# balkce/beamform

Measured on AMD Instinct MI355X. Metric: stft_frames_per_sec, higher is better.
Workload: dtype f64; 1 GPU; das 8-mic 1024-pt (hop 512), 65536-frame batch per GPU, 1 stream(s), planar input resident in HBM; frames_per_gpu=65536, frames_fed_per_gpu=65536, mics=8, fft=1024, hop=512, streams=1, layout=planar, gather=n/a, parallelism=independent batches x1, input=uniform noise in [-0.5, 0.5), settle_launches_before_warmup=408, forward_transforms_per_frame_pair=6

## Files before the change

beamform_amd/csrc/das_f64_w64.hip:

```cpp
#include <hip/hip_runtime.h>

#include <type_traits>

#include "launch_trace.hpp"
#include "pipeline_kernels.hpp"
#include "w64_f64_dev.hpp"

namespace bf {

namespace {

constexpr int kBlock = 512;
constexpr int kWaves = kBlock / 64;
constexpr int kHop = 512;
constexpr int kTwD = 2 * (1024 + 4 * kTw2RowW64Rot);
constexpr int oTw = 0;
constexpr int oPlane = kTwD;
constexpr int oGain = oPlane + kWaves * kPlaneD;
constexpr int oCross = oGain + 4 * 2048;
constexpr int oFlag = oCross + 512;
constexpr int kWinRow = 18;
constexpr int oWin = oFlag + 8;
constexpr int kLdsD = oWin + 64 * kWinRow;

// ... 218 lines not shown
            }
        } else {
            const float *parea = (pw < kWaves - 1) ? reinterpret_cast<const float *>(lds + oPlane + pw * kPlaneD) : s_cross + ((it + 1) & 1) * kHop;
            while (s_ready[pw] < (int)(t - 1)) __builtin_amdgcn_s_sleep(1);
            asm volatile("" ::: "memory");
            float prev[8];
#pragma unroll
            for (int j = 0; j < 8; ++j) prev[j] = parea[64 * j + lane];
            asm volatile("" ::: "memory");
            if (lane == 0) s_cons[pw] = (int)(t - 1);
#pragma unroll
            for (int j = 0; j < 8; ++j) yo[(unsigned)(64 * j + lane)] = prev[j] + o[j];
        }
        if (t == T1 - 1) {
            if (T1 < a.n_frames) {
                float *yn = ys + T1 * kHop;
#pragma unroll
                for (int j = 0; j < 8; ++j) atomicAdd(yn + (unsigned)(64 * j + lane), o[j + 8]);
            } else {
                float *to = a.tail_out + (long)stream * kHop;
#pragma unroll
                for (int j = 0; j < 8; ++j) to[(unsigned)(64 * j + lane)] = o[j + 8];
            }
        }
    }
}


#ifdef BF_PARK_PLAIN
#define BF_PARK_LD(p) (*(const volatile float *)(p))
#else
#define BF_PARK_LD(p) __builtin_nontemporal_load(p)
#endif
constexpr int kGRow = 65;
constexpr int kGMic = 8 * kGRow;
constexpr int kSlots = 64;
constexpr int kTwP = 2 * (960 + 4 * kTw2RowW64Rot);
constexpr int pTw = 0;
constexpr int pPlane = kTwP;
constexpr int pGain = pPlane + kWaves * kPlaneD;
constexpr int pFlag = pGain + 7 * kGMic * 2;
constexpr int kRingR = 32;
constexpr int kRingSlots = kRingR + kWaves;
constexpr int pRing = pFlag + (kSlots + 4) / 2;
constexpr int pWin = pRing + kRingR / 2;
constexpr int kLdsP = pWin + 64 * kWinRow;
static_assert(kLdsP * 8 <= 160 * 1024, "LDS");
static_assert((pGain & 1) == 0 && (pWin & 1) == 0, "16-byte alignment");


typedef volatile __attribute__((address_space(3))) int *lds_int_t;
typedef volatile __attribute__((address_space(3))) unsigned long long *lds_u64_t;
__device__ __forceinline__ int lds_fetch_add(lds_int_t p, int v, int lane) {
    int old = 0;
    if (lane == 0) old = __hip_atomic_fetch_add((__attribute__((address_space(3))) int *)p, v, __ATOMIC_RELAXED, __HIP_MEMORY_SCOPE_WORKGROUP);
    return __builtin_amdgcn_readfirstlane(old);
}
__device__ __forceinline__ unsigned long long lds_fetch_add64(lds_u64_t p, int lane) {
    unsigned long long old = 0;
    if (lane == 0) old = __hip_atomic_fetch_add((__attribute__((address_space(3))) unsigned long long *)p, 1ull, __ATOMIC_RELAXED, __HIP_MEMORY_SCOPE_WORKGROUP);
    const unsigned lo = (unsigned)__builtin_amdgcn_readfirstlane((int)(unsigned)old), hi = (unsigned)__builtin_amdgcn_readfirstlane((int)(unsigned)(old >> 32));
    return ((unsigned long long)hi << 32) | lo;
}
struct DasSched {
    const int4 *chunks;
    unsigned *counter;
    int n_chunks;
};
__device__ __forceinline__ unsigned long long pack_work(unsigned vbase, int chunk, int pairs, int next) {
    return ((unsigned long long)(vbase & 0xFFFFFFu) << 40) | ((unsigned long long)(unsigned)chunk << 20) | ((unsigned long long)(unsigned)pairs << 10) | (unsigned)next;
}
struct PairWork {
    int4 d;
    int pos;
    int len;
    unsigned u;
    bool have;
};
__device__ __forceinline__ int4 load_chunk(const int4 *chunks, int k) {
    const int4 d = chunks[k];
// ... 96 lines not shown
    __builtin_amdgcn_wave_barrier();
}

__device__ __forceinline__ float max3abs(float m, float x, float y) {
#if defined(__HIP_DEVICE_COMPILE__)
    float r;
    asm("v_max3_f32 %0, %1, |%2|, |%3|" : "=v"(r) : "v"(m), "v"(x), "v"(y));
    return r;
#else
    return fmaxf(m, fmaxf(fabsf(x), fabsf(y)));
#endif
}

template <int LAYOUT>
__device__ __forceinline__ void das_f64_pair_body(const DasF64Args &a, const DasSched &sc) {
    __shared__ __attribute__((aligned(16))) double lds[kLdsP];
    const cx<double> *s_tw1 = reinterpret_cast<const cx<double> *>(lds + pTw) - 64;
    const cx<double> *s_tw2 = reinterpret_cast<const cx<double> *>(lds + pTw) + 960;
    const cx<double> *s_gain = reinterpret_cast<const cx<double> *>(lds + pGain);
    lds_int_t s_state = (lds_int_t)(lds + pFlag);
    lds_u64_t s_work = (lds_u64_t)(lds + pFlag + kSlots / 2);
    lds_int_t s_ring = (lds_int_t)(lds + pRing);
    (void)s_ring;

    const int tid = threadIdx.x, lane = tid & 63;
    const int w = __builtin_amdgcn_readfirstlane(tid >> 6);
    const int M = a.n_mics;
    double *plane = lds + pPlane + w * kPlaneD;
    double *wcol = plane + w64_col_rot(lane);
    double *row16 = plane + (lane & 15) * kRS + 16 * (lane >> 4);
    const double *wrow = lds + pWin + lane * kWinRow;
    typedef double cxa __attribute__((ext_vector_type(2)));
    typedef const __attribute__((address_space(3))) cxa *lds_gain_t;
    unsigned gd0 = (unsigned)(size_t)(lds_gain_t)(s_gain + lane);
    asm volatile("" : "+v"(gd0));
    gd0 &= ~15u;
    const unsigned g_mirror = 2u * (unsigned)(size_t)(lds_gain_t)s_gain + 1024u;

    float n0[8], n1[8], n2[8];
#ifndef BF_PAIR_NT
#define BF_PAIR_NT 0
#endif
    auto request = [&](const float *h0, const float *h1, const float *h2) {
#pragma unroll
        for (int j = 0; j < 8; ++j) {
            n0[j] = (BF_PAIR_NT & 2) ? __builtin_nontemporal_load(h0 + (unsigned)(64 * j + lane)) : h0[(unsigned)(64 * j + lane)];
            n1[j] = (BF_PAIR_NT & 1) ? __builtin_nontemporal_load(h1 + (unsigned)(64 * j + lane)) : h1[(unsigned)(64 * j + lane)];
            n2[j] = (BF_PAIR_NT & 4) ? __builtin_nontemporal_load(h2 + (unsigned)(64 * j + lane)) : h2[(unsigned)(64 * j + lane)];
        }
    };
    auto request_pair_mic = [&](int stream, long tA, int m) {
        const float *h1 = a.x + (long)stream * a.stream_stride_x + (long)m * a.mic_stride + tA * kHop;
        const float *h0 = tA >= 1 ? h1 - kHop : a.hist + ((long)stream * M + m) * kHop;
        const float *h2 = tA + 1 < a.n_frames ? h1 + kHop : h1;
        request(h0, h1, h2);
    };
    float q0[8], q1[8], q2[8];
    const double inv_m = 1.0 / (double)M;
    float e0[8], e1[8], e2[8];
    const int NT = a.n_tr, XM = a.extra_mic;
    auto request_extra = [&](bool on, int stream, long tA) {
        if (!on) {
#pragma unroll
            for (int j = 0; j < 8; ++j) e0[j] = e1[j] = e2[j] = 0.f;
            return;
        }
        const float *h1 = a.x + (long)stream * a.stream_stride_x + (long)XM * a.mic_stride + tA * kHop;
        const float *h0 = tA >= 1 ? h1 - kHop : a.hist + ((long)stream * M + XM) * kHop;
        const float *h2 = tA + 1 < a.n_frames ? h1 + kHop : h1;
#pragma unroll
// ... 90 lines not shown
#pragma unroll
        for (int j = 0; j < 8; ++j) {
            e0[j] = r.h[XM * kHop + (unsigned)(64 * j + lane)];
            e1[j] = r.a[XM * kHop + (unsigned)(64 * j + lane)];
            e2[j] = r.b[XM * kHop + (unsigned)(64 * j + lane)];
        }
    };
    RingHops curR{nullptr, nullptr, nullptr};
    (void)curR;

    BF_STAMP(0);
#ifdef BF_W64_STAMPS
    if (lane == 0 && blockIdx.x < 256) g_stamps[(blockIdx.x * 8 + w) * 64 + 59] = __builtin_amdgcn_s_memtime();
#endif
    PairWork cur;
    cur.d = load_chunk(sc.chunks, (int)blockIdx.x);
    cur.len = (cur.d.z + 1) >> 1;
    const int n_static = cur.len < kWaves ? cur.len : kWaves;
    cur.pos = w;
    cur.u = (unsigned)w;
    cur.have = w < n_static;
    if (LAYOUT == 0 && cur.have) {
        request_pair_mic(cur.d.x, cur.d.y + 2L * w, a.slot_mic[0]);
        request_extra(XM >= 0, cur.d.x, cur.d.y + 2L * w);
    } else {
        request_extra(false, 0, 0);
    }
    {
        const f64x2 *tw2 = a.tw + 64;
        f64x2 *ltw = reinterpret_cast<f64x2 *>(lds + pTw), *lg = reinterpret_cast<f64x2 *>(lds + pGain);
#pragma unroll 4
        for (int i = tid; i < kTwP / 2; i += kBlock) ltw[i] = tw2[i];
        for (int k = 0; k < NT; ++k) {
            const f64x2 *g2 = a.gains_mic + a.slot_mic[k] * kGMic;
#pragma unroll 2
            for (int i = tid; i < kGMic; i += kBlock) lg[k * kGMic + i] = g2[i];
        }
#pragma unroll 2
        for (int i = tid; i < 1024; i += kBlock) lds[pWin + (i & 63) * kWinRow + (i >> 6)] = a.win[i];
        if (tid < kSlots) s_state[tid] = 0;
        if (tid < kRingR) s_ring[tid] = 0;
        if (tid == 0) *s_work = pack_work(0u, (int)blockIdx.x, cur.len, n_static);
    }
    __syncthreads();
    BF_STAMP(1);
    BF_STATS_DECL;
    int it = 0;
    if (!cur.have) {
        cur = draw_pair(s_work, sc, lane, cur.d);
        if (LAYOUT == 0 && cur.have) {
            request_pair_mic(cur.d.x, cur.d.y + 2L * cur.pos, a.slot_mic[0]);
            request_extra(XM >= 0, cur.d.x, cur.d.y + 2L * cur.pos);
        }
    }
    int mode = 0;
    PairWork nxt;
    nxt.have = false;
    nxt.d = int4{0, 0, 0, 0};
    nxt.pos = nxt.len = 0;
    nxt.u = 0;
    while (cur.have) {
        if constexpr (LAYOUT == 1) {
            if (mode == 0) curR = prepare_pair(cur);
            request_ring_mic(curR, a.slot_mic[0]);
            request_ring_extra(XM >= 0, curR);
        }
        const int stream = cur.d.x;
        const long T0 = cur.d.y, T1 = T0 + cur.d.z;
        const long tA = T0 + 2L * cur.pos;
// ... 60 lines not shown
                if (mode == 2) {
#pragma unroll
                    for (int j = 0; j < 16; ++j) re[j] = 0.0;
                } else {
#pragma unroll
                    for (int j = 0; j < 16; ++j) im[j] = 0.0;
                }
            }
            if (k + 1 < NT) {
                if constexpr (LAYOUT == 1) request_ring_mic(curR, a.slot_mic[k + 1]);
                else request_pair_mic(stream, tA, a.slot_mic[k + 1]);
            } else {
                if (mode == 0) nxt = draw_pair(s_work, sc, lane, cur.d);
                if constexpr (LAYOUT == 0) {
                    if (mode != 1) {
                        if (nxt.have) request_pair_mic(nxt.d.x, nxt.d.y + 2L * nxt.pos, a.slot_mic[0]);
                        else request_pair_mic(stream, tA, a.slot_mic[0]);
                    }
                }
            }
            cx<double> tw[15];
            BF_STAGE();
            load_tw1<1, 9>(tw, s_tw1, lane);
            BF_STAGE();
            fft16_core<double, -1, true, 1>(re, im);
            BF_STAGE();
            load_tw1<9, 16>(tw, s_tw1, lane);
            BF_STAGE();
            mul_tw<false, 1, 9>(re, im, tw);
            BF_STAGE();
            mul_tw<false, 9, 16>(re, im, tw);
            BF_STAGE();
            T1_fwd(re, im, wcol, row16);
            load_tw2<1, 9>(tw, s_tw2, lane);
            BF_STAGE();
            fft16_core<double, -1, true>(re, im);
            BF_STAGE();
            load_tw2<9, 16>(tw, s_tw2, lane);
            BF_STAGE();
            mul_tw<false, 1, 9>(re, im, tw);
            BF_STAGE();
            mul_tw<false, 9, 16>(re, im, tw);
            BF_STAGE();
            w64_T2_any<true>(re, im, row16 - 16 * (lane >> 4), lane >> 4);
            cxa g[16];
            const lds_gain_t gd = (lds_gain_t)(size_t)(gd0 + (unsigned)(k * kGMic * 16));
            const lds_gain_t gm = (lds_gain_t)(size_t)((g_mirror + (unsigned)(2 * k * kGMic * 16)) - (gd0 + (unsigned)(k * kGMic * 16)));
            BF_STAGE();
#pragma unroll
            for (int r = 0; r < 8; ++r)
                g[r] = (r & 3) < 2 ? gd[(2 * (r >> 2) + (r & 3)) * kGRow] : gm[(2 * (3 - (r >> 2)) + 3 - (r & 3)) * kGRow];
            BF_STAGE();
            w64_fwd_p3<double>(re, im);
            BF_STAGE();
#pragma unroll
            for (int r = 8; r < 16; ++r)
                g[r] = (r & 3) < 2 ? gd[(2 * (r >> 2) + (r & 3)) * kGRow] : gm[(2 * (3 - (r >> 2)) + 3 - (r & 3)) * kGRow];
            BF_STAGE();
#pragma unroll
            for (int r = 0; r < 16; ++r) {
                if (r == 8) BF_STAGE();
                const double gx = g[r].x, gy = (r & 3) < 2 ? g[r].y : -g[r].y;
                if constexpr (FIRST) {
                    Sr[r] = fma(-gy, im[r], gx * re[r]);
                    Si[r] = fma(gy, re[r], gx * im[r]);
                } else {
                    Sr[r] = fma(-gy, im[r], fma(gx, re[r], Sr[r]));
                    Si[r] = fma(gy, re[r], fma(gx, im[r], Si[r]));
                }
            }
        };
        auto request_own = [&]() {
            if constexpr (LAYOUT == 0) {
                request_pair_mic(stream, tA, a.slot_mic[0]);
                request_extra(XM >= 0, stream, tA);
            }
        };
        one_mic(0, std::true_type{});
        for (int k = 1; k < NT; ++k) one_mic(k, std::false_type{});
        if (mode == 0 && pair) {
            const unsigned b0 = wave_max_u32(__float_as_uint(hm0)), b1 = wave_max_u32(__float_as_uint(hm1)), b2 = wave_max_u32(__float_as_uint(hm2));
            const bool nan = __builtin_amdgcn_ballot_w64(hi_abs(Sr[0]) >= 0x7FF00000u || hi_abs(Si[0]) >= 0x7FF00000u) != 0;
            if (__builtin_expect(nan || !das_f64_may_pair(b0, b1, b2), 0)) {
                mode = 1;
                request_own();
                continue;
            }
        }
        const bool lone = !pair || mode == 1;
        float *yo = ys + tA * kHop;
        cx<double> tw[15];
        BF_STAGE();
        {
            const float *h0 = LAYOUT == 1 ? curR.h : (first_hop ? hist0 : hp0 - kHop), *h1 = LAYOUT == 1 ? curR.a : hp0;
            const float *h2 = LAYOUT == 1 ? curR.b : (last_hop ? hp0 : hp0 + kHop);
// ... 292 lines not shown
```

beamform_amd/csrc/geometry.hpp:

```cpp
#pragma once

#include <cmath>
#include <complex>
#include <vector>

#include "fft1024_w64.hpp"
#include "fft32.hpp"

namespace bf {

typedef std::complex<double> cplxd;

constexpr double kPi = 3.141592653589793238462643383279502884;
constexpr double kSoundSpeed = 343.0;

struct ArrayGeometry {
    int n_mics = 0;
    std::vector<double> dist;
    std::vector<double> ang_deg;

    void set(const double *x, const double *y, int n) {
        n_mics = n;
        dist.resize(n);
        ang_deg.resize(n);
// ... 173 lines not shown
            const double a = 2.0 * kPi * (double)((15 * b * k) % 64) / 64.0;
            t[1024 + b * kTw2RowW64Rot + k] = f64x2{std::cos(a), std::sin(a)};
        }
    return t;
}
inline std::vector<f64x2> das_pair_gains_w64_f64(const std::vector<f64x2> &D32, int n_pairs) {
    std::vector<f64x2> D((size_t)n_pairs * 1024);
    std::vector<f64x2> nat(1024);
    for (int p = 0; p < n_pairs; ++p) {
        for (int i = 0; i < 32; ++i)
            for (int l = 0; l < 32; ++l) nat[l + 32 * brev5(i)] = D32[((size_t)p * 32 + i) * 32 + l];
        for (int r = 0; r < 16; ++r)
            for (int l = 0; l < 64; ++l) D[((size_t)p * 16 + r) * 64 + l] = nat[w64_bin(l, r)];
    }
    return D;
}

constexpr int kDasMicGainRow = 65, kDasMicGainRows = 8;
inline std::vector<f64x2> das_mic_gains_w64_f64(const SteeringSet &s, int n_mics_alloc) {
    const int N = s.n_fft, M = s.n_mics;
    std::vector<f64x2> T((size_t)n_mics_alloc * kDasMicGainRows * kDasMicGainRow, f64x2{0, 0});
    for (int m = 0; m < M && m < n_mics_alloc; ++m)
        for (int g = 0; g < 4; ++g)
            for (int k3 = 0; k3 < 2; ++k3)
                for (int c = 0; c <= 64; ++c) {
                    const int k = 64 * g + 256 * k3 + c;
                    const cplxd c1 = std::conj(s.at(k, m, 0)) / (double)M, c2 = std::conj(s.at((N - k) % N, m, 0)) / (double)M;
                    const cplxd ce = 0.5 * (c1 + std::conj(c2)) / (double)N;
                    T[((size_t)m * kDasMicGainRows + 2 * g + k3) * kDasMicGainRow + c] = f64x2{ce.real(), ce.imag()};
                }
    return T;
}

struct DasSlots {
    int n_tr = 0, extra_mic = -1;
    int slot_mic[8] = {1, 2, 3, 4, 5, 6, 7, 0};
    bool mic0_unit = false;
};
inline DasSlots das_f64_slots(const SteeringSet &s) {
    DasSlots sl;
    const int N = s.n_fft, M = s.n_mics;
    if (M < 1 || M > 8) return sl;
    sl.mic0_unit = true;
    for (int j = 0; j < N && sl.mic0_unit; ++j) sl.mic0_unit = s.at(j, 0, 0) == cplxd(1.0, 0.0);
    auto same_row = [&](int a, int b) { int j = 0; while (j < N && s.at(j, a, 0) == s.at(j, b, 0)) ++j; return j == N; };
    int pa = -1;
    for (int a = 1; a < M && pa < 0; ++a)
        for (int b = a + 1; b < M && pa < 0; ++b)
            if (same_row(a, b)) { sl.slot_mic[sl.n_tr++] = pa = a; sl.extra_mic = b; }
    for (int m = 1; m < M; ++m)
        if (m != pa && m != sl.extra_mic) sl.slot_mic[sl.n_tr++] = m;
    return sl;
}

}
```

beamform_amd/csrc/pipeline.hip:

```cpp
#include "pipeline.hpp"

#include <hip/hip_runtime.h>

#include <cmath>
#include <utility>
#include <vector>

#include "device_mem.hpp"
#include "fft1024.hpp"
#include "pipeline_kernels.hpp"
#include "switches.hpp"

namespace bf {

namespace {

class BinPipelineImpl : public Engine {
    static constexpr int kMaxCols = BF_MAX_INTERF + 1;
   public:
    BinPipelineImpl(const bf_config &c, int n_cus) : cfg_(c), n_cus_(n_cus) {
        M_ = c.n_mics;
        H_ = c.hop;
        N_ = 2 * c.hop;
        NQ_ = problems_per_frame(N_);
// ... 28 lines not shown
            return BF_ENOSYS;
        }
        if (cov_node_ && (Phist_ < 1 || Phist_ > 64)) {
            err_ = "past_windows must be in 1..64";
            return BF_EINVAL;
        }
        if (time_node_ && (M_ > 16 || cfg_.gsc_filter_size < 1 || cfg_.gsc_filter_size > 256)) {
            err_ = "gsc is built for up to 16 microphones and filter_size 1..256";
            return M_ > 16 ? BF_ENOSYS : BF_EINVAL;
        }
        if (cfg_.algo == BF_PHASEMPF && (cfg_.smooth_size < 1 || cfg_.smooth_size > 64)) {
            err_ = "smooth_size must be in 1..64";
            return BF_EINVAL;
        }
        ENGINE_HIP(d_tw_.upload(N_ == 1024 ? twiddle_table_32x32<f64x2>() : stockham_twiddles<f64x2>(N_)));
        ENGINE_HIP(d_tw32_.upload(twiddle_table_32x32<f32x2>()));
        ENGINE_HIP(d_win_.upload(sqrt_hann(N_)));
        freqs_ = frequency_vector(N_, cfg_.sample_rate);
        ENGINE_HIP(d_freq_.upload(freqs_));
        skip_lo_ = N_; band_yh_hi_ = NQ_ - 1;
        if (band_node_) {
            int klo = N_, khi = 0;
            for (int q = 1; q < NQ_; ++q) {
                const double f = std::fabs(freqs_[q]);
                if (f >= cfg_.freq_min && f <= cfg_.freq_max) { if (q < klo) klo = q; khi = q; }
            }
            if (khi < N_ / 2 - 2) { skip_lo_ = khi; skip_hi_ = N_ - khi; }
            if (cov_node_ && khi < N_ / 2 - 1 && klo <= khi) { band_yh_lo_ = klo; band_yh_hi_ = khi; }
            else if (cov_node_ && klo > khi) { band_yh_lo_ = 1; band_yh_hi_ = 0; }
        }
        for (auto &b : d_steer_) ENGINE_HIP(b.alloc(steer_elems()));
        if (das_one_launch_shape()) {
            for (auto &t : das_) ENGINE_HIP(t.gains_w64.alloc((size_t)4 * 1024));
            for (auto &t : das_) ENGINE_HIP(t.gains_mic.alloc((size_t)8 * kDasMicGainRows * kDasMicGainRow));
            ENGINE_HIP(d_das_sched_.alloc(das_f64_sched_ws_bytes()));
        }
        if (N_ == 1024) ENGINE_HIP(d_tw_w64_.upload(twiddle_table_w64_rot()));
        for (auto &b : d_hist2_) ENGINE_HIP(b.alloc(hist_elems()));
        for (auto &b : d_tail_) ENGINE_HIP(b.alloc(tail_elems()));
        if (Phist_ > 0) ENGINE_HIP(d_zhist_.alloc(zhist_bytes()));
        if (cfg_.algo == BF_GSS) {
            ENGINE_HIP(d_gssW_.alloc(gss_bytes() / sizeof(f64x2)));
            ENGINE_HIP(hipMemset(d_gssW_.get(), 0, gss_bytes()));
        }
        if (mpf_bytes()) ENGINE_HIP(d_mpf_.alloc(mpf_bytes() / sizeof(double)));
        if (cfg_.algo == BF_PHASEMPF) ENGINE_HIP(d_smooth_.alloc(smooth_bytes() / sizeof(double)));
        if (time_node_) ENGINE_HIP(d_nlms_.alloc(nlms_bytes() / sizeof(float)));
        return BF_OK;
    }

    int reset(hipStream_t st) override {
        ENGINE_HIP(hipMemsetAsync(d_hist2_[0].get(), 0, hist_elems() * sizeof(float), st));
        hist_cur_ = 0;
        for (auto &b : d_tail_) ENGINE_HIP(hipMemsetAsync(b.get(), 0, tail_elems() * sizeof(float), st));
        tail_cur_ = 0;
        if (d_zhist_.get()) ENGINE_HIP(hipMemsetAsync(d_zhist_.get(), 0, zhist_bytes(), st));
        if (d_mpf_.get()) ENGINE_HIP(hipMemsetAsync(d_mpf_.get(), 0, mpf_bytes(), st));
        if (d_smooth_.get()) ENGINE_HIP(hipMemsetAsync(d_smooth_.get(), 0, smooth_bytes(), st));
        if (d_nlms_.get()) ENGINE_HIP(hipMemsetAsync(d_nlms_.get(), 0, nlms_bytes(), st));
        gss_reset_mask_ = ~0ull;
        if (d_gssW_.get()) ENGINE_HIP(hipMemsetAsync(d_gssW_.get(), 0, gss_bytes(), st));
        return BF_OK;
    }

    int upload_steering(const std::vector<SteeringSet> &dirs, hipStream_t stream) override {
        const int nc = dirs[0].n_cols, nd = (int)dirs.size();
        if ((size_t)nd * nc * M_ * N_ > steer_elems()) {
            err_ = "steering table larger than the device buffer";
            return BF_EINVAL;
        }
        std::vector<f64x2> t((size_t)nd * N_ * M_ * nc);
        for (int d = 0; d < nd; ++d)
            for (int c = 0; c < nc; ++c)
                for (int m = 0; m < M_; ++m)
                    for (int j = 0; j < N_; ++j) {
                        const cplxd w = dirs[d].at(j, m, c);
                        t[(((size_t)d * nc + c) * M_ + m) * N_ + j] = f64x2{w.real(), w.imag()};
                    }
        const int nxt = steer_cur_ ^ 1;
        std::vector<f64x2> dg64, dgm;
        if (das_one_launch_shape()) {
            dg64 = das_pair_gains_w64_f64(das_pair_gains_t<f64x2>(dirs[0], 4), 4);
            dgm = das_mic_gains_w64_f64(dirs[0], 8);
            das_[nxt].slots = das_f64_slots(dirs[0]);
            ENGINE_HIP(hipMemcpyAsync(das_[nxt].gains_w64.get(), dg64.data(), dg64.size() * sizeof(f64x2), hipMemcpyHostToDevice, stream));
            ENGINE_HIP(hipMemcpyAsync(das_[nxt].gains_mic.get(), dgm.data(), dgm.size() * sizeof(f64x2), hipMemcpyHostToDevice, stream));
        }
        ENGINE_HIP(hipMemcpyAsync(d_steer_[nxt].get(), t.data(), t.size() * sizeof(f64x2), hipMemcpyHostToDevice, stream));
        ENGINE_HIP(hipStreamSynchronize(stream));
        steer_cur_ = nxt;
        steer_dir_stride_ = (long)nc * M_ * N_;
        return BF_OK;
    }

    bool can_track() const override { return (cfg_.algo == BF_DAS || cfg_.algo == BF_PHASE || cfg_.algo == BF_PHASEMPF) && D_ == 1; }
    bool can_ctrack() const override { return cov_node_ && D_ == 1; }
    int install_track_tables(const std::vector<f64x2> &tables, int n_angles) override {
        if (!can_track() && !can_ctrack()) return Engine::install_track_tables(tables, n_angles);
        ENGINE_HIP(hipDeviceSynchronize());
        d_track_retired_ = std::move(d_track_);
        track_n_ = 0;
        if (n_angles > 0) {
            ENGINE_HIP(d_track_.upload(tables));
            track_n_ = n_angles;
        }
        return BF_OK;
    }

    void on_theta_changed(int dir) override { gss_reset_mask_ |= dir < 0 ? ~0ull : (1ull << dir); }
    void set_columns(int kp1) override {
        KP1_ = kp1;
        gss_reset_mask_ = ~0ull;
    }

    RunSnapshot snapshot_for_run() override {
        RunSnapshot sn;
        sn.kp1 = KP1_;
        sn.gss_reset_mask = gss_reset_mask_;
        sn.steer = d_steer_[steer_cur_].get();
        sn.steer_dir_stride = steer_dir_stride_;
        sn.das = DasSnapshot{das_[steer_cur_].gains_w64.get(), das_[steer_cur_].gains_mic.get(), das_[steer_cur_].slots};
        sn.track_tables = d_track_.get();
        sn.track_n = track_n_;
        gss_reset_mask_ = 0;
        return sn;
    }
    int columns() const override { return KP1_; }
    unsigned long long pending_resets() const override { return gss_reset_mask_; }
    void set_pending_resets(unsigned long long mask) override { gss_reset_mask_ = mask; }

    int run(const float *x, long F, float *y, f64x2 *spectrum, hipStream_t stream, int layout, long mic_stride,
            const RunSnapshot &snap) override;

    size_t state_bytes() const override {
        return (hist_elems() + tail_elems()) * sizeof(float) + zhist_bytes() + gss_bytes() + mpf_bytes() + smooth_bytes() +
               nlms_bytes();
    }
    int get_state(void *host) override { return copy_state((char *)host, true); }
    int set_state(const void *host) override { return copy_state((char *)host, false); }

   private:
    static constexpr int kDeclined = 1;
    int run_das_one_launch(const float *x, long F, float *y, hipStream_t stream, int layout, long mic_stride, const RunSnapshot &snap);
    int run_chain(const float *x, long F, float *y, f64x2 *spectrum, hipStream_t stream, int layout, long mic_stride, const RunSnapshot &snap);
    bool das_one_launch_shape() const { return cfg_.algo == BF_DAS && N_ == 1024 && M_ <= 8 && D_ == 1; }
    size_t steer_elems() const { return (size_t)D_ * N_ * M_ * kMaxCols; }
    size_t hist_elems() const { return (size_t)S_ * M_ * H_; }
    size_t tail_elems() const { return (size_t)So_ * R_ * H_; }
    size_t zhist_bytes() const { return Phist_ ? (size_t)S_ * Phist_ * NP_ * N_ * zsz_ : 0; }
    size_t gss_bytes() const { return cfg_.algo == BF_GSS ? (size_t)So_ * N_ * kMaxCols * M_ * sizeof(f64x2) : 0; }
    size_t mpf_bytes() const {
        if (post_filter_) return (size_t)So_ * R_ * (kMpfVecs * N_ + 8) * sizeof(double);
        return (cfg_.algo == BF_PHASEMPF || cfg_.algo == BF_MCRA) ? (size_t)So_ * (kMpfVecs * N_ + 8) * sizeof(double) : 0;
    }
// ... 10 lines not shown
            {d_nlms_.get(), nlms_bytes()}};
        for (auto &s : segs) {
            if (!s.n) continue;
            if (to_host)
                ENGINE_HIP(hipMemcpy(p, s.d, s.n, hipMemcpyDeviceToHost));
            else
                ENGINE_HIP(hipMemcpy(s.d, p, s.n, hipMemcpyHostToDevice));
            p += s.n;
        }
        return BF_OK;
    }

    bf_config cfg_;
    int n_cus_, M_, MF_, NP_, S_, D_, So_, R_, KP1_, Phist_;
    const bool cov_node_ = cfg_.algo == BF_MVDR || cfg_.algo == BF_LCMV;
    const bool band_node_ = cov_node_ || cfg_.algo == BF_GSS;
    const bool time_node_ = cfg_.algo == BF_GSC;
    const bool single_ch_ = cfg_.algo == BF_MCRA;
    const bool post_filter_ = cfg_.algo == BF_GSS && cfg_.gss_postfilter != 0;
    const bool post_amp_ = band_node_;
    const bool yraw_target_ = cfg_.algo == BF_PHASEMPF || time_node_;
    int skip_lo_, skip_hi_ = 0;
    int band_yh_lo_ = 0, band_yh_hi_;
    bool z48_ = false;
    size_t zsz_ = sizeof(f64x2);
    int H_ = 512, N_ = 1024, NQ_ = 514, YS_ = 516;
    const KernelSet *ks_ = nullptr;
    long steer_dir_stride_ = 0;
    std::vector<double> freqs_;
    DeviceBuffer<f64x2> d_tw_;
    DeviceBuffer<f32x2> d_tw32_;
    DeviceBuffer<double> d_win_, d_freq_;
    DeviceBuffer<f64x2> d_steer_[2];
    struct DasTables { DeviceBuffer<f64x2> gains_w64, gains_mic; DasSlots slots; } das_[2];
    DeviceBuffer<f64x2> d_tw_w64_;
    DeviceBuffer<char> d_das_sched_;
    int steer_cur_ = 0;
    DeviceBuffer<f64x2> d_track_;
    DeviceBuffer<f64x2> d_track_retired_;
    int track_n_ = 0;
    DeviceBuffer<float> d_hist2_[2];
    int hist_cur_ = 0;
    DeviceBuffer<float> d_tail_[2];
    int tail_cur_ = 0;
    DeviceBuffer<char> d_zhist_;
    DeviceBuffer<f64x2> d_gssW_;
    DeviceBuffer<double> d_mpf_;
    DeviceBuffer<double> d_smooth_;
    DeviceBuffer<float> d_nlms_;
    unsigned long long gss_reset_mask_ = ~0ull;
    DeviceBuffer<char> d_Z_;
    DeviceBuffer<char> d_Yh_;
    DeviceBuffer<float> d_yraw_;
    DeviceBuffer<float> d_planar_;
    DeviceBuffer<float> d_frames_;
};

int BinPipelineImpl::run_das_one_launch(const float *x, long F, float *y, hipStream_t stream, int layout, long mic_stride, const RunSnapshot &snap) {
    const Switches &sw = switches();
    if (!das_one_launch_shape() || sw.fused_bins != 1 || snap.das.gains_w64 == nullptr) return kDeclined;
    const DasSlots &sl = snap.das.slots;
    const DasF64Launch d = das_f64_decide(DasF64Shape{layout, M_, S_, n_cus_, F, sl.mic0_unit, snap.das.gains_mic && d_das_sched_.get(), sl.n_tr,
                                                      sw.das_il_ring, sw.das_f64_sched});
    if (d.path == DasF64Path::kChain) return kDeclined;
    ENGINE_HIP(d_planar_.reserve((d.scratch_bytes + sizeof(float) - 1) / sizeof(float)));
    float *const hist = d_hist2_[hist_cur_].get();
    DasF64Args da;
    da.x = x; da.hist = hist; da.hist_out = d_hist2_[hist_cur_ ^ 1].get(); da.y = y;
    da.tail_in = d_tail_[tail_cur_].get(); da.tail_out = d_tail_[tail_cur_ ^ 1].get();
    da.win = d_win_.get(); da.n_frames = F; da.mic_stride = mic_stride;
    da.stream_stride_x = (long)M_ * F * H_; da.n_streams = S_; da.n_mics = M_; da.run_len = 1; da.layout = layout;
    da.gains = snap.das.gains_w64; da.gains_mic = snap.das.gains_mic; da.tw = d_tw_w64_.get();
    da.mic0_unit = sl.mic0_unit ? 1 : 0; da.n_tr = sl.n_tr; da.extra_mic = sl.extra_mic;
    for (int k = 0; k < 8; ++k) da.slot_mic[k] = sl.slot_mic[k];
    da.sched_ws = d_das_sched_.get(); da.sched_ws_bytes = d_das_sched_.get() ? das_f64_sched_ws_bytes() : 0;
    ENGINE_HIP(enqueue_das_f64(da, d, d_planar_.get(), stream, kev0, kev1, &kev_recorded));
    if (d.writes_hist)
        hist_cur_ ^= 1;
    else
        ENGINE_HIP(carry_last_hop(hist, x, F, H_, M_, S_, layout, mic_stride, (long)F * H_ * M_, stream));
    tail_cur_ ^= 1;
    return BF_OK;
}

int BinPipelineImpl::run(const float *x, long F, float *y, f64x2 *spectrum, hipStream_t stream, int layout, long mic_stride,
                         const RunSnapshot &snap) {
    const int rc = (spectrum || snap.track) ? kDeclined : run_das_one_launch(x, F, y, stream, layout, mic_stride, snap);
    return rc == kDeclined ? run_chain(x, F, y, spectrum, stream, layout, mic_stride, snap) : rc;
}

int BinPipelineImpl::run_chain(const float *x, long F, float *y, f64x2 *spectrum, hipStream_t stream, int layout, long mic_stride,
                               const RunSnapshot &snap) {
    const Switches &sw = switches();
    const ChainPlan p = chain_decide(ChainShape{cfg_.algo, N_, layout, M_, S_, cfg_.n_dirs > 1 ? cfg_.n_dirs : 1, snap.kp1, cfg_.past_windows,
                                                cfg_.precision, spectrum != nullptr, F, n_cus_, cfg_.gsc_filter_size, cfg_.smooth_size,
                                                band_yh_lo_, band_yh_hi_, (reinterpret_cast<size_t>(y) & 15) == 0, sw.fused_bins,
                                                sw.stft_small, sw.stft_split, sw.mvdr_group, sw.gss_group, sw.gsc_serial, cfg_.algo == BF_GSS ? R_ : 1, snap.track != nullptr && snap.track_cols == 0,
                                                snap.track != nullptr ? snap.track_cols : 0, post_filter_ ? 1 : 0, cfg_.algo == BF_LCMV ? R_ : 1});
    float *const hist = d_hist2_[hist_cur_].get();
    const long FT = Phist_ + F;
    ENGINE_HIP(d_Z_.reserve(p.z_bytes));
    ENGINE_HIP(d_Yh_.reserve(p.yh_bytes));
    ENGINE_HIP(d_yraw_.reserve(p.yraw_elems));
    ENGINE_HIP(d_frames_.reserve(p.frames_elems));
    f64x2 *const Z = (f64x2 *)d_Z_.get();
// ... 80 lines not shown
```

beamform_amd/csrc/pipeline.hpp:

```cpp
#pragma once

#include <hip/hip_runtime.h>

#include <cstdint>
#include <string>
#include <vector>

#include "../../include/bfcore.h"
#include "geometry.hpp"

namespace bf {

struct DasSnapshot {
    const f64x2 *gains_w64 = nullptr, *gains_mic = nullptr;
    DasSlots slots;
};

struct RunSnapshot {
    int kp1 = 1;
    unsigned long long gss_reset_mask = 0;
    const f64x2 *steer = nullptr;
    long steer_dir_stride = 0;
    DasSnapshot das;
    const f64x2 *track_tables = nullptr;
    int track_n = 0;
    const int32_t *track = nullptr;
    int track_cols = 0;
};

class Engine {
   public:
    static Engine *create(const bf_config &cfg, int n_cus);
    virtual ~Engine() {}
    virtual int init() = 0;
    virtual int reset(hipStream_t stream) = 0;
    virtual int upload_steering(const std::vector<SteeringSet> &dirs, hipStream_t stream) = 0;
    virtual void on_theta_changed(int dir = -1) = 0;
    virtual void set_columns(int kp1) = 0;
    virtual bool can_track() const { return false; }
    virtual bool can_ctrack() const { return false; }
    virtual int install_track_tables(const std::vector<f64x2> &, int) {
        err_ = "steering tracks: das in double, phase and phasempf with one look direction";
        return BF_ENOSYS;
    }
    virtual RunSnapshot snapshot_for_run() = 0;
    virtual int run(const float *x_dev, long n_frames, float *y_dev, f64x2 *spectrum_dev, hipStream_t stream, int layout,
                    long mic_stride, const RunSnapshot &snap) = 0;
// ... 27 lines not shown
```

beamform_amd/csrc/pipeline_kernels.hpp:

```cpp
#pragma once

#include <hip/hip_runtime.h>

#include <cstdint>

#include "../../include/bfcore.h"
#include "chain_plan.hpp"
#include "das_f64_plan.hpp"
#include "geometry.hpp"

namespace bf {

#ifdef BF_NFFT
#define BF_CAT2_(a, b) a##b
#define BF_CAT2(a, b) BF_CAT2_(a, b)
#define BF_NTAG BF_CAT2(n, BF_NFFT)
#endif

constexpr int problems_per_frame(int nfft) { return nfft / 2 + 2; }
constexpr int yh_stride(int nfft) { return nfft / 2 + 4; }
constexpr int kMpfVecs = 7;
#ifdef BF_NFFT
namespace BF_NTAG {
constexpr int kN = BF_NFFT;
// ... 56 lines not shown
    long track_stride = 0;
};
struct IstftArgs {
    const f64x2 *Yh;
    int yh32;
    int yh_lo, yh_hi;
    float *y;
    const float *tail_in;
    float *tail_out;
    const f64x2 *tw;
    const f32x2 *tw32;
    const f64x2 *tw_w64 = nullptr;
    float *frames;
    const double *win;
    long n_frames;
    int n_streams;
    double post_amp;
    int use_post_amp;
    int pair_span = 20;
};
struct DasF64Args {
    const float *x;
    const float *hist;
    float *y;
    const float *tail_in;
    float *tail_out;
    const f64x2 *gains;
    const f64x2 *tw;
    const double *win;
    long n_frames, mic_stride, stream_stride_x;
    int n_streams, n_mics, run_len;
    int layout = 0;
    float *hist_out = nullptr;
    const f64x2 *gains_mic = nullptr;
    int n_tr = 0, extra_mic = -1;
    int slot_mic[8] = {1, 2, 3, 4, 5, 6, 7, 0};
    int mic0_unit = 0;
    void *sched_ws = nullptr;
    size_t sched_ws_bytes = 0;
    float *ring = nullptr;
    size_t ring_bytes = 0;
};

hipError_t enqueue_das_f64(DasF64Args a, const DasF64Launch &d, float *scratch, hipStream_t s, hipEvent_t kev0, hipEvent_t kev1, bool *kev_recorded);

#ifdef BF_NFFT
namespace BF_NTAG {
hipError_t launch_stft(const ChainPlan &p, const StftArgs &a, int n_cus, hipStream_t s);
hipError_t launch_bins(const ChainPlan &p, const BinsArgs &a, int n_cus, hipStream_t s);
hipError_t launch_stft_bins_fused(const ChainPlan &p, const StftArgs &a, const BinsArgs &b, int n_cus, hipStream_t s);
hipError_t launch_pointwise(const ChainPlan &p, const BinsArgs &a, hipStream_t s);
hipError_t launch_mpf_mask(const ChainPlan &p, const BinsArgs &a, hipStream_t s);
hipError_t launch_mcra_node(const BinsArgs &a, hipStream_t s);
hipError_t launch_mvdr_lcmv(const ChainPlan &p, const BinsArgs &a, int n_cus, hipStream_t s);
hipError_t launch_gss(const ChainPlan &p, const BinsArgs &a, hipStream_t s);
hipError_t launch_gsc_align(const BinsArgs &a, hipStream_t s);
hipError_t launch_bins_end(const ChainPlan &p, const BinsArgs &a, hipStream_t s);
hipError_t launch_gss_postfilter(const ChainPlan &p, const BinsArgs &a, hipStream_t s);
hipError_t launch_expand_spectrum(const f64x2 *Yh, f64x2 *spectrum, long frames, hipStream_t s);
hipError_t launch_istft(const ChainPlan &p, const IstftArgs &a, int n_cus, hipStream_t s);
hipError_t launch_gsc_nlms(const ChainPlan &p, const float *aligned, float *y, float *state, long n_samples, int n_streams, int n_mics,
                           const bf_config &cfg, hipStream_t s);
hipError_t launch_smooth(const ChainPlan &p, const float *yraw, float *y, double *state, long n_frames, int n_streams, hipStream_t s);
}
#endif

struct KernelSet {
// ... 31 lines not shown
```

Baseline: 133.5 million frames/s.

## Factor per-mic DAS steering gains into separable tables folded into FFT twiddles

Replaces the dense per-mic gain table, about 520 complex entries per mic, with a separable factorization. One factor is folded into per-mic second-stage twiddles. The per-bin gain then comes from a small 4x16 table, with two exception rows for registers 2 and 13. This shrinks the LDS footprint and gain loads per frame, removes the mirrored-conjugate indexing, and loads twiddles from the per-mic table instead of the shared one. The host checks the factorization's error against a bound and falls back to the other path if it fails, which adds rounding risk and host precompute.

```diff
diff --git a/beamform_amd/csrc/das_f64_w64.hip b/beamform_amd/csrc/das_f64_w64.hip
--- a/beamform_amd/csrc/das_f64_w64.hip
+++ b/beamform_amd/csrc/das_f64_w64.hip
@@ -274,20 +274,20 @@
 #else
 #define BF_PARK_LD(p) __builtin_nontemporal_load(p)
 #endif
-constexpr int kGRow = 65;
-constexpr int kGMic = 8 * kGRow;
+constexpr int kGSlot = kDasSepMic;
 constexpr int kSlots = 64;
 constexpr int kTwP = 2 * (960 + 4 * kTw2RowW64Rot);
 constexpr int pTw = 0;
 constexpr int pPlane = kTwP;
 constexpr int pGain = pPlane + kWaves * kPlaneD;
-constexpr int pFlag = pGain + 7 * kGMic * 2;
+constexpr int pFlag = pGain + 7 * kGSlot * 2;
 constexpr int kRingR = 32;
 constexpr int kRingSlots = kRingR + kWaves;
 constexpr int pRing = pFlag + (kSlots + 4) / 2;
 constexpr int pWin = pRing + kRingR / 2;
 constexpr int kLdsP = pWin + 64 * kWinRow;
-static_assert(kLdsP * 8 <= 160 * 1024, "LDS");
+static_assert(kLdsP * 8 <= 120 * 1024, "LDS");
+static_assert(kGSlot <= kBlock, "a slot's table is copied into LDS in one trip of the block");
 static_assert((pGain & 1) == 0 && (pWin & 1) == 0, "16-byte alignment");
 
 
@@ -450,10 +450,11 @@
     const double *wrow = lds + pWin + lane * kWinRow;
     typedef double cxa __attribute__((ext_vector_type(2)));
     typedef const __attribute__((address_space(3))) cxa *lds_gain_t;
-    unsigned gd0 = (unsigned)(size_t)(lds_gain_t)(s_gain + lane);
-    asm volatile("" : "+v"(gd0));
-    gd0 &= ~15u;
-    const unsigned g_mirror = 2u * (unsigned)(size_t)(lds_gain_t)s_gain + 1024u;
+    unsigned gG0 = (unsigned)(size_t)(lds_gain_t)(s_gain + kDasSepG + (lane & 15));
+    unsigned gE0 = (unsigned)(size_t)(lds_gain_t)(s_gain + kDasSepE13 + lane);
+    unsigned gT0 = (unsigned)(size_t)(lds_gain_t)(s_gain + kDasSepTw2 + (lane >> 4) * kTw2RowW64Rot);
+    asm volatile("" : "+v"(gG0), "+v"(gE0), "+v"(gT0));
+    gG0 &= ~15u; gE0 &= ~15u; gT0 &= ~15u;
 
     float n0[8], n1[8], n2[8];
 #ifndef BF_PAIR_NT
@@ -610,9 +611,8 @@
 #pragma unroll 4
         for (int i = tid; i < kTwP / 2; i += kBlock) ltw[i] = tw2[i];
         for (int k = 0; k < NT; ++k) {
-            const f64x2 *g2 = a.gains_mic + a.slot_mic[k] * kGMic;
-#pragma unroll 2
-            for (int i = tid; i < kGMic; i += kBlock) lg[k * kGMic + i] = g2[i];
+            const f64x2 *g2 = a.gains_sep + a.slot_mic[k] * kGSlot;
+            if (tid < kGSlot) lg[k * kGSlot + tid] = g2[tid];
         }
 #pragma unroll 2
         for (int i = tid; i < 1024; i += kBlock) lds[pWin + (i & 63) * kWinRow + (i >> 6)] = a.win[i];
@@ -739,35 +739,36 @@
             mul_tw<false, 9, 16>(re, im, tw);
             BF_STAGE();
             T1_fwd(re, im, wcol, row16);
-            load_tw2<1, 9>(tw, s_tw2, lane);
+            const lds_gain_t gt = (lds_gain_t)(size_t)(gT0 + (unsigned)(k * kGSlot * 16));
+#pragma unroll
+            for (int i = 1; i < 9; ++i) { const cxa v = gt[brev4(i)]; tw[i - 1] = cx<double>{v.x, v.y}; }
             BF_STAGE();
             fft16_core<double, -1, true>(re, im);
             BF_STAGE();
-            load_tw2<9, 16>(tw, s_tw2, lane);
+#pragma unroll
+            for (int i = 9; i < 16; ++i) { const cxa v = gt[brev4(i)]; tw[i - 1] = cx<double>{v.x, v.y}; }
             BF_STAGE();
             mul_tw<false, 1, 9>(re, im, tw);
             BF_STAGE();
             mul_tw<false, 9, 16>(re, im, tw);
             BF_STAGE();
             w64_T2_any<true>(re, im, row16 - 16 * (lane >> 4), lane >> 4);
-            cxa g[16];
-            const lds_gain_t gd = (lds_gain_t)(size_t)(gd0 + (unsigned)(k * kGMic * 16));
-            const lds_gain_t gm = (lds_gain_t)(size_t)((g_mirror + (unsigned)(2 * k * kGMic * 16)) - (gd0 + (unsigned)(k * kGMic * 16)));
-            BF_STAGE();
-#pragma unroll
-            for (int r = 0; r < 8; ++r)
-                g[r] = (r & 3) < 2 ? gd[(2 * (r >> 2) + (r & 3)) * kGRow] : gm[(2 * (3 - (r >> 2)) + 3 - (r & 3)) * kGRow];
+            cxa g[4], g13, g2;
+            const lds_gain_t gd = (lds_gain_t)(size_t)(gG0 + (unsigned)(k * kGSlot * 16));
+            const lds_gain_t ge = (lds_gain_t)(size_t)(gE0 + (unsigned)(k * kGSlot * 16));
+            BF_STAGE();
+#pragma unroll
+            for (int k3 = 0; k3 < 4; ++k3) g[k3] = gd[16 * k3];
+            g13 = ge[0];
+            g2 = ge[kDasSepE2 - kDasSepE13];
             BF_STAGE();
             w64_fwd_p3<double>(re, im);
-            BF_STAGE();
-#pragma unroll
-            for (int r = 8; r < 16; ++r)
-                g[r] = (r & 3) < 2 ? gd[(2 * (r >> 2) + (r & 3)) * kGRow] : gm[(2 * (3 - (r >> 2)) + 3 - (r & 3)) * kGRow];
             BF_STAGE();
 #pragma unroll
             for (int r = 0; r < 16; ++r) {
                 if (r == 8) BF_STAGE();
-                const double gx = g[r].x, gy = (r & 3) < 2 ? g[r].y : -g[r].y;
+                const cxa gr = r == 13 ? g13 : r == 2 ? g2 : g[r & 3];
+                const double gx = gr.x, gy = gr.y;
                 if constexpr (FIRST) {
                     Sr[r] = fma(-gy, im[r], gx * re[r]);
                     Si[r] = fma(gy, re[r], gx * im[r]);
diff --git a/beamform_amd/csrc/geometry.hpp b/beamform_amd/csrc/geometry.hpp
--- a/beamform_amd/csrc/geometry.hpp
+++ b/beamform_amd/csrc/geometry.hpp
@@ -229,6 +229,60 @@
     return T;
 }
 
+constexpr int kDasSepG = 0, kDasSepE13 = 64, kDasSepE2 = 128, kDasSepTw2 = 192, kDasSepMic = 192 + 4 * kTw2RowW64Rot;
+struct DasSepTables {
+    std::vector<f64x2> t;
+    bool ok = false;
+    double bound = 0.0, worst = 0.0;
+};
+inline DasSepTables das_sep_gains_w64_f64(const SteeringSet &s, const std::vector<f64x2> &T , int n_mics_alloc) {
+    typedef std::complex<long double> cl;
+    const int N = s.n_fft, M = s.n_mics;
+    DasSepTables r;
+    r.t.assign((size_t)n_mics_alloc * kDasSepMic, f64x2{0, 0});
+    if (N != 1024 || M < 1) return r;
+    const long double scale = 1.0L / ((long double)M * (long double)N);
+    const std::vector<f64x2> tw2 = twiddle_table_w64_rot();
+    auto wl = [&](int k, int m) { const cplxd w = s.at(k, m, 0); return cl((long double)w.real(), -(long double)w.imag()); };
+    auto tab = [&](int m, int k) -> cl {
+        const int kk = k <= 512 ? k : N - k, k3 = kk >= 512 ? 1 : (kk >> 8) & 1, g = kk >= 512 ? 3 : (kk >> 6) & 3, c = kk - 64 * g - 256 * k3;
+        const f64x2 v = T[((size_t)m * kDasMicGainRows + 2 * g + k3) * kDasMicGainRow + c];
+        return cl((long double)v.x, k <= 512 ? (long double)v.y : -(long double)v.y);
+    };
+    auto rnd = [](cl v) { return f64x2{(double)v.real(), (double)v.imag()}; };
+    r.ok = true;
+    for (int m = 1; m < M && m < n_mics_alloc; ++m) {
+        f64x2 *t = r.t.data() + (size_t)m * kDasSepMic;
+        cl B[16];
+        for (int k2 = 0; k2 < 16; ++k2) B[k2] = wl(16 * k2, m);
+        const cl C3 = wl(768, m), C[4] = {cl(1.0L, 0.0L), wl(256, m), C3 * C3, C3};
+        for (int k3 = 0; k3 < 4; ++k3)
+            for (int k1 = 0; k1 < 16; ++k1) t[kDasSepG + 16 * k3 + k1] = rnd(wl(k1, m) * C[k3] * scale);
+        for (int l = 0; l < 64; ++l) {
+            t[kDasSepE13 + l] = rnd(tab(m, 448 + l) / B[12 + (l >> 4)]);
+            t[kDasSepE2 + l] = rnd(tab(m, 512 + l) / B[l >> 4]);
+        }
+        for (int b = 0; b < 4; ++b)
+            for (int k2 = 0; k2 < 16; ++k2) {
+                const f64x2 w2 = tw2[1024 + b * kTw2RowW64Rot + k2];
+                t[kDasSepTw2 + b * kTw2RowW64Rot + k2] = rnd(cl((long double)w2.x, (long double)w2.y) * B[k2]);
+            }
+        const cplxd w1 = s.at(1, m, 0);
+        const double bound = (16.0 + 12.0 * 512.0 * std::fabs(std::atan2(w1.imag(), w1.real()))) * 0x1p-53;
+        if (bound > r.bound) r.bound = bound;
+        for (int k = 0; k < N; ++k) {
+            const int k1 = k & 15, k2 = (k >> 4) & 15, k3 = k >> 8, l = k & 63, reg = 4 * (k2 >> 2) + k3;
+            const f64x2 gv = reg == 13 ? t[kDasSepE13 + l] : reg == 2 ? t[kDasSepE2 + l] : t[kDasSepG + 16 * k3 + k1];
+            const f64x2 bv = rnd(B[k2]);
+            const cl d = cl((long double)gv.x, (long double)gv.y) * cl((long double)bv.x, (long double)bv.y) - tab(m, k);
+            const double dev = (double)(std::abs(d) / scale);
+            if (!(dev <= bound)) r.ok = false;
+            if (dev > r.worst || dev != dev) r.worst = dev;
+        }
+    }
+    return r;
+}
+
 struct DasSlots {
     int n_tr = 0, extra_mic = -1;
     int slot_mic[8] = {1, 2, 3, 4, 5, 6, 7, 0};
diff --git a/beamform_amd/csrc/pipeline.hip b/beamform_amd/csrc/pipeline.hip
--- a/beamform_amd/csrc/pipeline.hip
+++ b/beamform_amd/csrc/pipeline.hip
@@ -84,7 +84,7 @@
         for (auto &b : d_steer_) ENGINE_HIP(b.alloc(steer_elems()));
         if (das_one_launch_shape()) {
             for (auto &t : das_) ENGINE_HIP(t.gains_w64.alloc((size_t)4 * 1024));
-            for (auto &t : das_) ENGINE_HIP(t.gains_mic.alloc((size_t)8 * kDasMicGainRows * kDasMicGainRow));
+            for (auto &t : das_) ENGINE_HIP(t.gains_sep.alloc((size_t)8 * kDasSepMic));
             ENGINE_HIP(d_das_sched_.alloc(das_f64_sched_ws_bytes()));
         }
         if (N_ == 1024) ENGINE_HIP(d_tw_w64_.upload(twiddle_table_w64_rot()));
@@ -131,12 +131,15 @@
                     }
         const int nxt = steer_cur_ ^ 1;
         std::vector<f64x2> dg64, dgm;
+        DasSepTables sep;
         if (das_one_launch_shape()) {
             dg64 = das_pair_gains_w64_f64(das_pair_gains_t<f64x2>(dirs[0], 4), 4);
             dgm = das_mic_gains_w64_f64(dirs[0], 8);
             das_[nxt].slots = das_f64_slots(dirs[0]);
+            sep = das_sep_gains_w64_f64(dirs[0], dgm, 8);
+            das_[nxt].sep_ok = sep.ok; das_[nxt].sep_bound = sep.bound; das_[nxt].sep_worst = sep.worst;
+            ENGINE_HIP(hipMemcpyAsync(das_[nxt].gains_sep.get(), sep.t.data(), sep.t.size() * sizeof(f64x2), hipMemcpyHostToDevice, stream));
             ENGINE_HIP(hipMemcpyAsync(das_[nxt].gains_w64.get(), dg64.data(), dg64.size() * sizeof(f64x2), hipMemcpyHostToDevice, stream));
-            ENGINE_HIP(hipMemcpyAsync(das_[nxt].gains_mic.get(), dgm.data(), dgm.size() * sizeof(f64x2), hipMemcpyHostToDevice, stream));
         }
         ENGINE_HIP(hipMemcpyAsync(d_steer_[nxt].get(), t.data(), t.size() * sizeof(f64x2), hipMemcpyHostToDevice, stream));
         ENGINE_HIP(hipStreamSynchronize(stream));
@@ -171,7 +174,8 @@
         sn.gss_reset_mask = gss_reset_mask_;
         sn.steer = d_steer_[steer_cur_].get();
         sn.steer_dir_stride = steer_dir_stride_;
-        sn.das = DasSnapshot{das_[steer_cur_].gains_w64.get(), das_[steer_cur_].gains_mic.get(), das_[steer_cur_].slots};
+        sn.das = DasSnapshot{das_[steer_cur_].gains_w64.get(),
+                             das_[steer_cur_].sep_ok ? das_[steer_cur_].gains_sep.get() : nullptr, das_[steer_cur_].slots};
         sn.track_tables = d_track_.get();
         sn.track_n = track_n_;
         gss_reset_mask_ = 0;
@@ -248,7 +252,7 @@
     DeviceBuffer<f32x2> d_tw32_;
     DeviceBuffer<double> d_win_, d_freq_;
     DeviceBuffer<f64x2> d_steer_[2];
-    struct DasTables { DeviceBuffer<f64x2> gains_w64, gains_mic; DasSlots slots; } das_[2];
+    struct DasTables { DeviceBuffer<f64x2> gains_w64, gains_sep; DasSlots slots; bool sep_ok = false; double sep_bound = 0.0, sep_worst = 0.0; } das_[2];
     DeviceBuffer<f64x2> d_tw_w64_;
     DeviceBuffer<char> d_das_sched_;
     int steer_cur_ = 0;
@@ -276,7 +280,7 @@
     const Switches &sw = switches();
     if (!das_one_launch_shape() || sw.fused_bins != 1 || snap.das.gains_w64 == nullptr) return kDeclined;
     const DasSlots &sl = snap.das.slots;
-    const DasF64Launch d = das_f64_decide(DasF64Shape{layout, M_, S_, n_cus_, F, sl.mic0_unit, snap.das.gains_mic && d_das_sched_.get(), sl.n_tr,
+    const DasF64Launch d = das_f64_decide(DasF64Shape{layout, M_, S_, n_cus_, F, sl.mic0_unit, snap.das.gains_sep && d_das_sched_.get(), sl.n_tr,
                                                       sw.das_il_ring, sw.das_f64_sched});
     if (d.path == DasF64Path::kChain) return kDeclined;
     ENGINE_HIP(d_planar_.reserve((d.scratch_bytes + sizeof(float) - 1) / sizeof(float)));
@@ -286,7 +290,7 @@
     da.tail_in = d_tail_[tail_cur_].get(); da.tail_out = d_tail_[tail_cur_ ^ 1].get();
     da.win = d_win_.get(); da.n_frames = F; da.mic_stride = mic_stride;
     da.stream_stride_x = (long)M_ * F * H_; da.n_streams = S_; da.n_mics = M_; da.run_len = 1; da.layout = layout;
-    da.gains = snap.das.gains_w64; da.gains_mic = snap.das.gains_mic; da.tw = d_tw_w64_.get();
+    da.gains = snap.das.gains_w64; da.gains_sep = snap.das.gains_sep; da.tw = d_tw_w64_.get();
     da.mic0_unit = sl.mic0_unit ? 1 : 0; da.n_tr = sl.n_tr; da.extra_mic = sl.extra_mic;
     for (int k = 0; k < 8; ++k) da.slot_mic[k] = sl.slot_mic[k];
     da.sched_ws = d_das_sched_.get(); da.sched_ws_bytes = d_das_sched_.get() ? das_f64_sched_ws_bytes() : 0;
diff --git a/beamform_amd/csrc/pipeline.hpp b/beamform_amd/csrc/pipeline.hpp
--- a/beamform_amd/csrc/pipeline.hpp
+++ b/beamform_amd/csrc/pipeline.hpp
@@ -12,7 +12,7 @@
 namespace bf {
 
 struct DasSnapshot {
-    const f64x2 *gains_w64 = nullptr, *gains_mic = nullptr;
+    const f64x2 *gains_w64 = nullptr, *gains_sep = nullptr;
     DasSlots slots;
 };
 
diff --git a/beamform_amd/csrc/pipeline_kernels.hpp b/beamform_amd/csrc/pipeline_kernels.hpp
--- a/beamform_amd/csrc/pipeline_kernels.hpp
+++ b/beamform_amd/csrc/pipeline_kernels.hpp
@@ -112,7 +112,7 @@
     int n_streams, n_mics, run_len;
     int layout = 0;
     float *hist_out = nullptr;
-    const f64x2 *gains_mic = nullptr;
+    const f64x2 *gains_sep = nullptr;
     int n_tr = 0, extra_mic = -1;
     int slot_mic[8] = {1, 2, 3, 4, 5, 6, 7, 0};
     int mic0_unit = 0;
```

Measured after the change: 135.8 million frames/s (median of 6 runs). 1.7% higher.
